# xiexh20/CHORE

Measured on AMD Instinct MI355X. Metric: query-points/sec (HGFilters encode + 20k-pt MLP field query per 512x512 image), higher is better.
Workload: dtype fp16x3; 1 GPU; BASELINE configs[1]: encode 4x(5,512,512) + query 4x20000 points per GPU per step; images_per_gpu=4, points_per_image=20000, batches_in_flight=2

## Files before the change

chore_amd/_lib.py:

```python
import ctypes
import os

import torch
from ctypes import POINTER, c_char_p, c_float, c_int, c_int64, c_longlong, c_size_t, c_uint8, c_void_p

_HERE = os.path.dirname(os.path.abspath(__file__))
LIB_PATH = os.environ.get("CHORE_HIP_LIB") or os.path.join(_HERE, "csrc", "libchore_hip.so")

F32, BF16, F16X3, F16 = 0, 1, 2, 3
HEADS_X3 = 0x100


class WeightDesc(ctypes.Structure):
    _fields_ = [("name", c_char_p), ("ptr", c_void_p), ("numel", c_int64)]


class EncoderCfg(ctypes.Structure):
    _fields_ = [("in_channels", c_int), ("num_stack", c_int), ("num_hourglass", c_int),
                ("hourglass_dim", c_int)]


SIGNATURES = {
    "chore_version": (c_int, []),
    "chore_create": (c_int, [POINTER(c_void_p), c_int]),
    "chore_destroy": (c_int, [c_void_p]),
    "chore_last_error": (c_char_p, [c_void_p]),
    "chore_cu_count": (c_int, [c_void_p]),
    "chore_stream_create_cu_mask": (c_int, [c_void_p, POINTER(ctypes.c_uint32), c_int, POINTER(c_void_p)]),
    "chore_stream_destroy": (c_int, [c_void_p, c_void_p]),
    "chore_heads_arena_bytes": (c_size_t, [c_int]),
    "chore_heads_pack": (c_int, [c_void_p, POINTER(WeightDesc), c_int, c_int, c_void_p, c_void_p]),
    "chore_query_fwd": (c_int, [c_void_p, c_void_p, c_void_p, c_int, c_int,
                                c_void_p, c_int, c_int, c_void_p, c_int, c_int, c_int,
                                c_void_p, POINTER(c_float), c_void_p, c_void_p, c_void_p, c_void_p,
                                c_void_p, c_void_p]),
    "chore_query_fwd_workspace_bytes": (c_size_t, [c_int, c_int]),
    "chore_query_fwd_ws": (c_int, [c_void_p, c_void_p, c_void_p, c_int, c_int,
                                   c_void_p, c_int, c_int, c_void_p, c_int, c_int, c_int,
                                   c_void_p, POINTER(c_float), c_void_p, c_void_p, c_void_p, c_void_p,
                                   c_void_p, c_void_p, c_void_p]),
    "chore_sample_features": (c_int, [c_void_p, c_void_p, c_void_p, c_int, c_int,
                                      c_void_p, c_int, c_int, c_void_p, c_int, c_int, c_int,
                                      POINTER(c_float), c_void_p, c_void_p, c_void_p, c_void_p]),
    "chore_query_bwd_points": (c_int, [c_void_p, c_void_p, c_void_p, c_int, c_int,
                                       c_void_p, c_int, c_int, c_void_p, c_int, c_int, c_int,
                                       c_void_p, POINTER(c_float), c_void_p, c_void_p, c_void_p,
                                       c_void_p, c_void_p, c_void_p]),
    "chore_query_train_bytes": (c_size_t, [c_int, c_int]),
    "chore_query_fwd_train": (c_int, [c_void_p, c_void_p, c_void_p, c_int, c_int,
                                      c_void_p, c_int, c_int, c_void_p, c_int, c_int, c_int,
                                      c_void_p, POINTER(c_float), c_void_p, c_void_p, c_void_p, c_void_p,
                                      c_void_p, c_void_p, c_void_p]),
    "chore_query_bwd_train": (c_int, [c_void_p, c_void_p, c_void_p, c_int, c_int,
                                      c_void_p, c_int, c_int, c_void_p, c_int, c_int, c_int,
                                      c_void_p, POINTER(c_float), c_void_p, c_void_p, c_void_p,
                                      c_void_p, c_void_p, c_void_p, c_int, c_void_p]),
    "chore_scatter_features": (c_int, [c_void_p, c_void_p, c_void_p, c_int, c_int, c_int, c_int, c_int, c_int,
                                       POINTER(c_float), c_void_p, c_void_p, c_void_p, c_int, c_void_p]),
    "chore_encoder_arena_bytes": (c_size_t, [POINTER(EncoderCfg), c_int]),
    "chore_encoder_pack": (c_int, [c_void_p, POINTER(EncoderCfg), POINTER(WeightDesc), c_int, c_int,
                                   c_void_p, c_void_p]),
    "chore_encoder_workspace_bytes": (c_size_t, [POINTER(EncoderCfg), c_int, c_int, c_int, c_int]),
    "chore_encode_fwd": (c_int, [c_void_p, POINTER(EncoderCfg), c_void_p, c_int, c_int, c_int, c_int,
                                 c_void_p, c_void_p, c_size_t, POINTER(c_void_p), c_int, c_void_p,
                                 c_void_p, c_void_p]),
    "chore_smpl_arena_bytes": (c_size_t, [c_int, c_int, c_int]),
    "chore_smpl_workspace_bytes": (c_size_t, [c_int, c_int, c_int, c_int]),
    "chore_smpl_pack": (c_int, [c_void_p, c_int, c_int, c_int, c_void_p, c_void_p, c_void_p, c_void_p, c_void_p,
                                POINTER(c_int), c_void_p, c_void_p]),
    "chore_smpl_lbs_fwd": (c_int, [c_void_p, c_void_p, c_int, c_int, c_int, c_void_p, c_void_p, c_void_p, c_void_p,
                                   c_float, c_int, c_void_p, c_void_p, c_void_p, c_void_p, c_void_p, c_void_p]),
    "chore_smpl_lbs_bwd": (c_int, [c_void_p, c_void_p, c_int, c_int, c_int, c_void_p, c_float, c_int, c_void_p,
                                   c_void_p, c_void_p, c_void_p, c_void_p, c_void_p, c_void_p, c_void_p]),
    "chore_landmarks_fwd": (c_int, [c_void_p, c_void_p, c_void_p, c_int, c_int, c_int, c_void_p, c_void_p]),
    "chore_landmarks_bwd": (c_int, [c_void_p, c_void_p, c_void_p, c_int, c_int, c_int, c_void_p, c_void_p]),
    "chore_so3_aux_bytes": (c_size_t, [c_int]),
    "chore_so3_project_fwd": (c_int, [c_void_p, c_void_p, c_int, c_void_p, c_void_p, c_void_p]),
    "chore_so3_project_bwd": (c_int, [c_void_p, c_void_p, c_void_p, c_int, c_void_p, c_void_p]),
    "chore_conv2d_workspace_bytes": (c_size_t, [c_int, c_int, c_int, c_int]),
    "chore_gn_stats_bytes": (c_size_t, [c_int]),
    "chore_gn_stats": (c_int, [c_void_p, c_int, c_void_p, c_int, c_int, c_int, c_void_p, c_int, c_void_p]),
    "chore_gn_relu_fwd": (c_int, [c_void_p, c_int, c_void_p, c_void_p, c_void_p, c_void_p, c_void_p, c_int, c_int, c_int,
                                  c_void_p]),
    "chore_conv2d_fwd": (c_int, [c_void_p, c_int, c_int, c_void_p, c_int, c_int, c_int, c_int, c_void_p, c_void_p,
                                 c_void_p, c_void_p, c_void_p, c_int, c_void_p, c_void_p, c_void_p, c_void_p]),
    "chore_conv2d_pool_fwd": (c_int, [c_void_p, c_int, c_int, c_void_p, c_int, c_int, c_int, c_int, c_void_p, c_void_p,
                                      c_void_p, c_void_p, c_void_p, c_int, c_void_p, c_void_p, c_void_p, c_void_p, c_void_p,
                                      c_void_p, c_void_p]),
    "chore_amax_bytes": (c_size_t, []),
    "chore_absmax_f32": (c_int, [c_void_p, c_void_p, c_size_t, c_void_p, c_void_p]),
    "chore_conv2d_bwd_data": (c_int, [c_void_p, c_int, c_int, c_void_p, c_int, c_int, c_int, c_int, c_void_p, c_int,
                                      c_void_p, c_void_p, c_void_p, c_void_p]),
    "chore_conv2d_wgrad_workspace_bytes": (c_size_t, [c_int, c_int, c_int, c_int, c_int, c_int]),
    "chore_conv2d_bwd_weight": (c_int, [c_void_p, c_int, c_int, c_void_p, c_int, c_int, c_int, c_int, c_void_p, c_void_p,
                                        c_void_p, c_void_p, c_int, c_void_p, c_void_p, c_void_p, c_void_p, c_void_p]),
    "chore_convblock_saved_bytes": (c_size_t, [c_int, c_int, c_int, c_int, c_int, c_int]),
    "chore_convblock_out_stats_offset": (c_size_t, [c_int]),
    "chore_convblock_workspace_bytes": (c_size_t, [c_int, c_int, c_int, c_int, c_int, c_int]),
    "chore_convblock_grad_floats": (c_size_t, [c_int, c_int]),
    "chore_convblock_fwd": (c_int, [c_void_p, c_int, c_void_p, c_void_p, c_int, c_int, c_int, c_int, c_int, c_void_p, c_void_p,
                                    c_void_p, c_void_p, c_void_p, c_void_p, c_void_p, c_void_p, c_void_p]),
    "chore_convblock_bwd": (c_int, [c_void_p, c_int, c_void_p, c_void_p, c_void_p, c_int, c_int, c_int, c_int, c_int, c_void_p,
                                    c_void_p, c_void_p, c_void_p, c_void_p, c_void_p, c_void_p, c_void_p, c_void_p, c_void_p]),
    "chore_debug_nan_counts": (c_int, [c_void_p]),
    "chore_debug_last_conv": (c_int, [c_void_p, POINTER(c_int), c_int]),
    "chore_debug_last_wgrad": (c_int, [c_void_p, POINTER(c_int), c_int]),
    "chore_query_plan": (c_int, [c_int] * 9 + [POINTER(c_int), c_int]),
    "chore_conv_plan": (c_int, [c_int] * 9 + [POINTER(c_int), c_int]),
    "chore_fit_adam_step": (c_int, [c_void_p, c_void_p, c_void_p, c_void_p, c_void_p, c_void_p, c_int, c_void_p, c_float, c_float,
                                    c_float, c_float, c_void_p, c_void_p]),
    "chore_fit_adam_step_acc": (c_int, [c_void_p, c_void_p, c_void_p, c_void_p, c_void_p, c_void_p, c_void_p, c_void_p, c_void_p, c_int,
                                        c_void_p, c_float, c_float, c_float, c_float, c_void_p, c_int, c_void_p]),
    "chore_fit_weighted_sum_step": (c_int, [c_void_p, c_void_p, c_void_p, c_int, c_void_p, c_void_p, c_void_p, c_void_p, c_void_p, c_void_p,
                                            c_void_p, c_void_p, c_float, c_void_p, c_void_p, c_void_p]),
    "chore_fit_weighted_sum": (c_int, [c_void_p, c_void_p, c_void_p, c_int, c_void_p, c_void_p, c_void_p]),
    "chore_fit_weighted_sum_bwd": (c_int, [c_void_p, c_void_p, c_int, c_void_p, c_void_p, c_void_p, c_void_p]),
    "chore_fit_smpl_terms_fwd": (c_int, [c_void_p] * 11 + [c_int, c_int, c_int, c_void_p, c_void_p, c_void_p]),
    "chore_fit_smpl_terms_bwd": (c_int, [c_void_p] * 11 + [c_int, c_int, c_int, c_void_p, c_void_p, c_void_p, c_void_p, c_void_p]),
    "chore_fit_point_terms_workspace_bytes": (c_size_t, [c_int, c_int]),
    "chore_fit_point_terms_fwd": (c_int, [c_void_p, c_void_p, c_int, c_float, c_void_p, c_void_p, c_int, c_int, c_int, c_void_p,
                                          c_void_p, c_void_p, c_void_p]),
    "chore_fit_point_terms_bwd": (c_int, [c_void_p, c_void_p, c_int, c_float, c_void_p, c_void_p, c_int, c_int, c_int, c_void_p,
                                          c_void_p, c_void_p, c_void_p, c_void_p]),
    "chore_fit_obj_transform_fwd": (c_int, [c_void_p] * 5 + [c_int, c_int, c_void_p, c_void_p]),
    "chore_fit_obj_transform_bwd": (c_int, [c_void_p] * 6 + [c_int, c_int, c_void_p, c_void_p, c_void_p, c_void_p]),
    "chore_fit_obj_terms_workspace_bytes": (c_size_t, [c_int]),
    "chore_fit_obj_terms_fwd": (c_int, [c_void_p] * 5 + [c_float, c_int, c_int, c_void_p, c_void_p, c_void_p, c_void_p, c_void_p]),
    "chore_fit_obj_terms_bwd": (c_int, [c_void_p, c_void_p, c_void_p, c_float, c_void_p, c_void_p, c_int, c_int, c_void_p, c_void_p,
                                        c_void_p, c_void_p]),
    "chore_fit_rot_noise": (c_int, [c_void_p, c_void_p, c_void_p, c_void_p, c_float, c_int, c_longlong, c_void_p, c_void_p]),
    "chore_fit_stop_rule": (c_int, [c_void_p, c_void_p, c_void_p, c_void_p, c_void_p, c_float, c_void_p, c_void_p, c_void_p]),
    "chore_train_loss_workspace_bytes": (c_size_t, []),
    "chore_train_loss": (c_int, [c_void_p] * 11 + [c_int, c_int, c_float, c_void_p, c_float] + [c_void_p] * 5 + [c_int, c_void_p,
                                                                                                               c_void_p]),
    "chore_upadd_fwd": (c_int, [c_void_p, c_int, c_void_p, c_void_p, c_void_p, c_int, c_int, c_int, c_int, c_void_p, c_void_p]),
    "chore_up2_bwd": (c_int, [c_void_p, c_int, c_void_p, c_void_p, c_int, c_int, c_int, c_int, c_void_p]),
    "chore_avgpool2_fwd": (c_int, [c_void_p, c_int, c_void_p, c_void_p, c_int, c_int, c_int, c_int, c_void_p, c_void_p]),
    "chore_avgpool2_bwd": (c_int, [c_void_p, c_int, c_void_p, c_void_p, c_int, c_int, c_int, c_int, c_void_p]),
    "chore_stem_workspace_bytes": (c_size_t, [c_int]),
    "chore_stem_fwd": (c_int, [c_void_p, c_int, c_void_p, c_int, c_int, c_int, c_int, c_void_p, c_void_p, c_void_p, c_void_p,
                               c_void_p]),
    "chore_stem_x3_workspace_bytes": (c_size_t, [c_int]),
    "chore_stem_x3_fwd": (c_int, [c_void_p, c_void_p, c_int, c_int, c_int, c_int, c_void_p, c_void_p, c_void_p, c_void_p, c_void_p,
                                  c_void_p]),
    "chore_stem_wgrad_workspace_bytes": (c_size_t, [c_int, c_int, c_int, c_int]),
    "chore_stem_bwd_weight": (c_int, [c_void_p, c_int, c_void_p, c_int, c_int, c_int, c_int, c_void_p, c_void_p, c_void_p,
                                      c_void_p, c_void_p]),
    "chore_heads_wgrad_floats": (c_size_t, []),
    "chore_heads_wgrad_workspace_bytes": (c_size_t, []),
    "chore_heads_wgrad": (c_int, [c_void_p, c_void_p, c_int, c_int, c_void_p, c_void_p, c_void_p, c_void_p, c_void_p, c_void_p,
                                  c_int, c_void_p]),
    "chore_gemm_tn_workspace_bytes": (c_size_t, [c_int, c_int, c_int]),
    "chore_gemm_tn_f32": (c_int, [c_void_p, c_void_p, c_int, c_void_p, c_int, c_int, c_int, c_int, c_void_p, c_void_p,
                                  c_void_p]),
    "chore_gn_relu_bwd_workspace_bytes": (c_size_t, [c_int, c_int]),
    "chore_gn_relu_bwd": (c_int, [c_void_p, c_int, c_void_p, c_void_p, c_void_p, c_void_p, c_void_p, c_int, c_int, c_int,
                                  c_void_p, c_void_p, c_void_p, c_void_p, c_int, c_void_p]),
    "chore_eval_chamfer_workspace_bytes": (c_size_t, [c_int, c_int]),
    "chore_eval_chamfer": (c_int, [c_void_p, c_void_p, c_int, c_void_p, c_int, c_void_p, c_void_p, c_void_p]),
    "chore_eval_procrustes": (c_int, [c_void_p, c_void_p, c_void_p, c_int, c_void_p, c_void_p]),
    "chore_eval_apply_similarity": (c_int, [c_void_p, c_void_p, c_int, c_void_p, c_void_p, c_void_p]),
    "chore_gen_clamp_mask": (c_int, [c_void_p, c_void_p, c_int, c_float, c_int, c_int, c_void_p, c_void_p]),
    "chore_gen_surface_step": (c_int, [c_void_p, c_void_p, c_void_p, c_void_p, c_int, c_float, c_int, c_int, c_void_p, c_void_p]),
    "chore_gen_surface_step_fused": (c_int, [c_void_p, c_void_p, c_void_p, c_int, c_int, c_void_p, c_int, c_int, c_void_p, c_int, c_int,
                                             c_int, c_void_p, POINTER(c_float), c_int, c_float, c_void_p, c_void_p]),
    "chore_gen_compact": (c_int, [c_void_p, c_void_p, c_int, c_int, c_void_p, c_void_p, c_void_p]),
# ... 160 lines not shown
```

chore_amd/csrc/enc_misc.hip:

```cpp
#include "enc_common.h"
#include <type_traits>
#include <cstdlib>

constexpr int STEM_T = 16;
constexpr int STEM_P = 2 * STEM_T + 5;
constexpr int STEM_MAXC = 8;

template <typename T>
__global__ __launch_bounds__(256) void stem_kernel(const float* __restrict__ img, int B, int Cin, int H, int W,
                                                   const float* __restrict__ wk, const float* __restrict__ bias,
                                                   T* __restrict__ out) {
    extern __shared__ __attribute__((aligned(16))) float sm[];
    float* patch = sm;
    const int OH = H / 2, OW = W / 2;
    const int b = blockIdx.z, ty0 = blockIdx.y * STEM_T, tx0 = blockIdx.x * STEM_T;
    const int tid = threadIdx.x;
    const int iy0 = 2 * ty0 - 3, ix0 = 2 * tx0 - 3;
    for (int i = tid; i < Cin * STEM_P * STEM_P; i += 256) {
        const int c = i / (STEM_P * STEM_P), r = i % (STEM_P * STEM_P);
        const int y = iy0 + r / STEM_P, x = ix0 + r % STEM_P;
        float v = 0.f;
        if (y >= 0 && y < H && x >= 0 && x < W) v = img[(((size_t)b * Cin + c) * H + y) * W + x];
        patch[i] = v;
    }
// ... 334 lines not shown
                           st);
    CHORE_LAUNCH_CHECK(h, s);
    return CHORE_OK;
}

template <typename T, bool STATS>
__global__ __launch_bounds__(256) void gn_apply_relu_kernel(const T* __restrict__ x, int xcs, int xco,
                                                            const GroupStat* __restrict__ st,
                                                            const float* __restrict__ gamma,
                                                            const float* __restrict__ beta, T* __restrict__ y,
                                                            int ycs, int yco, int C, int HW, GroupStat* __restrict__ st_out) {
    __shared__ float ss[512];
    __shared__ float red[STATS ? 2 : 1][STATS ? 1024 : 1];
    const int b = blockIdx.y, tid = threadIdx.x;
    if (tid < C) gn_scale_shift(st, (int)gridDim.y, b, C, tid, HW, gamma, beta, ss[2 * tid], ss[2 * tid + 1]);
    __syncthreads();
    const int tpr = C / 4;
    const size_t total4 = (size_t)HW * tpr;
    f32x4 sum = {0.f, 0.f, 0.f, 0.f}, sq = {0.f, 0.f, 0.f, 0.f};
    for (size_t i = (size_t)blockIdx.x * 256 + tid; i < total4; i += (size_t)gridDim.x * 256) {
        const int cv = (int)(i % tpr);
        const size_t p = (size_t)b * HW + i / tpr;
        const f32x4 v = Vec4<T>::ld(x + p * xcs + xco + cv * 4);
        f32x4 r;
#pragma unroll
        for (int j = 0; j < 4; ++j) {
            const float t = fmaf(v[j], ss[2 * (cv * 4 + j)], ss[2 * (cv * 4 + j) + 1]);
            r[j] = t > 0.f ? t : 0.f;
        }
        if constexpr (STATS) {
            const f32x4 w = Vec4<T>::st_round(y + p * ycs + yco + cv * 4, r);
            sum += w;
            sq += w * w;
        } else Vec4<T>::st(y + p * ycs + yco + cv * 4, r);
    }
    if constexpr (STATS) {
        const int cv = tid % tpr, pl = tid / tpr, P = 256 / tpr;
#pragma unroll
        for (int j = 0; j < 4; ++j) {
            red[0][pl * C + cv * 4 + j] = sum[j];
            red[1][pl * C + cv * 4 + j] = sq[j];
        }
        __syncthreads();
        if (tid < C) {
            float a = 0.f, q = 0.f;
            for (int i = 0; i < P; ++i) { a += red[0][i * C + tid]; q += red[1][i * C + tid]; }
            const int gs = C / GN_GROUPS;
            a = group_lane_sum(a, gs);
            q = group_lane_sum(q, gs);
            GroupStat* o = st_out + (size_t)b * GN_GROUPS + tid / gs;
            if (tid % gs == 0) stat_add(&o->sum, act_hi_cells((int)gridDim.y), a);
            if (tid % gs == (gs > 1 ? 1 : 0)) stat_add(&o->sq, act_hi_cells((int)gridDim.y), q);
        }
    }
}

int launch_gn_apply_relu(chore_handle* h, int dtype, const View& x, const GroupStat* st, const float* gamma,
                         const float* beta, const View& y, int B, int HW, hipStream_t s, GroupStat* st_out) {
    if (!gn_channels_ok(x.C)) CHORE_FAIL(h, CHORE_EINVAL, "gn: unsupported C=%d", x.C);
    const size_t total4 = (size_t)HW * (x.C / 4);
    int blocks = (int)((total4 + 255) / 256);
    if (blocks > 1024) blocks = 1024;
    if (st_out) {
        if (256 % (x.C / 4)) CHORE_FAIL(h, CHORE_EINVAL, "gn_apply_relu with statistics: unsupported C=%d", x.C);
        if (blocks > 256) blocks = 256;
    }
    dim3 grid(blocks, B);
#define GN_APPLY(T, ST) hipLaunchKernelGGL((gn_apply_relu_kernel<T, ST>), grid, dim3(256), 0, s, (const T*)x.p, x.cs, x.co, st, gamma, beta, \
                                            (T*)y.p, y.cs, y.co, x.C, HW, st_out)
    if (dtype == CHORE_F16) { if (st_out) GN_APPLY(h16_t, true); else GN_APPLY(h16_t, false); }
    else if (dtype == CHORE_F32) { if (st_out) GN_APPLY(float, true); else GN_APPLY(float, false); }
    else { if (st_out) GN_APPLY(bf16_t, true); else GN_APPLY(bf16_t, false); }
#undef GN_APPLY
    CHORE_LAUNCH_CHECK(h, s);
    return CHORE_OK;
}

constexpr int MAP_T = 8;

template <typename T, int C> struct PoolOp {
    const T* x; int xcs, xco, H, W;
    static constexpr size_t SMEM = 0;
    static constexpr int CT = C, TW = MAP_T;
    __device__ __forceinline__ void stage(char*, int, int, int, int, int, int) const {}
    __device__ __forceinline__ void column(const char*, int b, int oy0, int ox, int, int c0, int cv, int OH,
                                           f32x4 (&out)[MAP_T]) const {
#pragma unroll
        for (int r = 0; r < MAP_T; ++r) {
            const int oy = oy0 + r < OH ? oy0 + r : OH - 1;
            const T* src = x + (((size_t)b * H + 2 * oy) * W + 2 * ox) * xcs + xco + c0 + cv * 4;
            const f32x4 a = Vec4<T>::ld(src), bb = Vec4<T>::ld(src + xcs);
            const f32x4 c = Vec4<T>::ld(src + (size_t)W * xcs), d = Vec4<T>::ld(src + (size_t)W * xcs + xcs);
            out[r] = (((a + bb) + c) + d) * 0.25f;
        }
    }
};

__device__ __forceinline__ void cubic_coeffs(float t, float (&c)[4]) {
    const float A = -0.75f;
    const float x0 = t + 1.0f, x1 = t, x2 = 1.0f - t, x3 = 2.0f - t;
    c[0] = ((A * x0 - 5.0f * A) * x0 + 8.0f * A) * x0 - 4.0f * A;
    c[1] = ((A + 2.0f) * x1 - (A + 3.0f)) * x1 * x1 + 1.0f;
    c[2] = ((A + 2.0f) * x2 - (A + 3.0f)) * x2 * x2 + 1.0f;
    c[3] = ((A * x3 - 5.0f * A) * x3 + 8.0f * A) * x3 - 4.0f * A;
}
template <typename T, int C> struct UpAddOp {
    static constexpr int CT = 64, TW = 16;
    static constexpr int PS = 8, PSX = TW / 2 + 4;
    static constexpr int TPR = CT / 4, P = 256 / TPR;
    static constexpr size_t SMEM = (size_t)PS * PSX * CT * sizeof(T);
    static_assert(C % CT == 0 && (PS * PSX) % P == 0 && TW % P == 0, "upadd tile geometry");
    const T* a; int acs, aco;
    const T* low; int lcs, lco, H, W;
    __device__ __forceinline__ float scale_y() const { return (float)(H - 1) / (float)(2 * H - 1); }
    __device__ __forceinline__ float scale_x() const { return (float)(W - 1) / (float)(2 * W - 1); }
    __device__ __forceinline__ void stage(char* sm, int b, int oy0, int ox0, int c0, int cv, int pl) const {
        const int iy0 = (int)floorf(scale_y() * (float)oy0) - 1, ix0 = (int)floorf(scale_x() * (float)ox0) - 1;
        constexpr int N = PS * PSX / P;
        typedef typename std::conditional<sizeof(T) == 2, unsigned long long, f32x4>::type Raw;
        Raw v[N];
#pragma unroll
        for (int i = 0; i < N; ++i) {
            const int q = pl + i * P;
            int yy = iy0 + q / PSX, xx = ix0 + q % PSX;
            yy = yy < 0 ? 0 : (yy > H - 1 ? H - 1 : yy);
            xx = xx < 0 ? 0 : (xx > W - 1 ? W - 1 : xx);
            v[i] = *(const Raw*)(low + (((size_t)b * H + yy) * W + xx) * lcs + lco + c0 + cv * 4);
        }
#pragma unroll
        for (int i = 0; i < N; ++i) *(Raw*)((T*)sm + (size_t)(pl + i * P) * CT + cv * 4) = v[i];
    }
    __device__ __forceinline__ void column(const char* sm, int b, int oy0, int ox, int ox0, int c0, int cv, int OH,
                                           f32x4 (&out)[MAP_T]) const {
        const int OW = 2 * W;
        const int iy0 = (int)floorf(scale_y() * (float)oy0) - 1, ix0 = (int)floorf(scale_x() * (float)ox0) - 1;
        f32x4 av[MAP_T];
#pragma unroll
        for (int r = 0; r < MAP_T; ++r) {
            const int oy = oy0 + r < OH ? oy0 + r : OH - 1;
            av[r] = Vec4<T>::ld(a + (((size_t)b * 2 * H + oy) * OW + ox) * acs + aco + c0 + cv * 4);
        }
        const float rx = scale_x() * (float)ox, fx = floorf(rx);
        const int kx = (int)fx - 1 - ix0;
        float cx[4];
        cubic_coeffs(rx - fx, cx);
        f32x4 rows[PS];
#pragma unroll
        for (int k = 0; k < PS; ++k) {
            const T* pr = (const T*)sm + (size_t)(k * PSX + kx) * CT + cv * 4;
            f32x4 acc = Vec4<T>::ld(pr) * cx[0];
#pragma unroll
            for (int q = 1; q < 4; ++q) {
                const f32x4 v = Vec4<T>::ld(pr + (size_t)q * CT);
#pragma unroll
                for (int e = 0; e < 4; ++e) acc[e] = fmaf(v[e], cx[q], acc[e]);
            }
            rows[k] = acc;
        }
#pragma unroll
        for (int r = 0; r < MAP_T; ++r) {
            const int oy = oy0 + r < OH ? oy0 + r : OH - 1;
            const float ry = scale_y() * (float)oy, fy = floorf(ry);
            const int ky = (int)fy - 1 - iy0;
            float cy[4];
            cubic_coeffs(ry - fy, cy);
            f32x4 acc = {0.f, 0.f, 0.f, 0.f};
            bool first = true;
#pragma unroll
            for (int k = 0; k < PS; ++k) {
                const int j = k - ky;
                if (j >= 0 && j < 4) {
                    const float w = cy[j];
#pragma unroll
                    for (int e = 0; e < 4; ++e) acc[e] = first ? rows[k][e] * w : fmaf(rows[k][e], w, acc[e]);
                    first = false;
                }
            }
            out[r] = av[r] + acc;
        }
    }
};

template <typename T, int C, typename Op>
__global__ __launch_bounds__(256) void map_stats_kernel(Op op, T* y, int ycs, int yco, int OH, int OW,
                                                        GroupStat* __restrict__ st) {
    extern __shared__ __attribute__((aligned(16))) char map_sm[];
    __shared__ float red[2][1024];
    constexpr int CT = Op::CT, TW = Op::TW;
    constexpr int TPR = CT / 4, P = 256 / TPR;
    static_assert(P * CT <= 1024, "partial-sum scratch");
    const int b = blockIdx.y, tid = threadIdx.x, c0 = blockIdx.z * CT;
    const int cv = tid % TPR, pl = tid / TPR;
    const int tiles_x = (OW + TW - 1) / TW;
    const int oy0 = (blockIdx.x / tiles_x) * MAP_T, ox0 = (blockIdx.x % tiles_x) * TW;
    op.stage(map_sm, b, oy0, ox0, c0, cv, pl);
    __syncthreads();
    f32x4 sum = {0.f, 0.f, 0.f, 0.f}, sq = {0.f, 0.f, 0.f, 0.f};
#pragma unroll
    for (int col = pl; col < TW; col += P) {
        const int ox = ox0 + col;
        if (ox < OW) {
            f32x4 out[MAP_T];
            op.column(map_sm, b, oy0, ox, ox0, c0, cv, OH, out);
#pragma unroll
            for (int r = 0; r < MAP_T; ++r) {
                const int oy = oy0 + r;
                if (oy < OH) {
                    const f32x4 v = Vec4<T>::st_round(y + (((size_t)b * OH + oy) * OW + ox) * ycs + yco + c0 + cv * 4, out[r]);
                    sum += v;
                    sq += v * v;
                }
            }
        }
    }
    if (!st) return;
#pragma unroll
    for (int j = 0; j < 4; ++j) {
        red[0][pl * CT + cv * 4 + j] = sum[j];
        red[1][pl * CT + cv * 4 + j] = sq[j];
    }
    __syncthreads();
    if (tid < CT) {
        float a = 0.f, q = 0.f;
#pragma unroll
        for (int i = 0; i < P; ++i) { a += red[0][i * CT + tid]; q += red[1][i * CT + tid]; }
        constexpr int gs = C / GN_GROUPS;
        static_assert(CT % gs == 0, "a channel slice holds whole GroupNorm groups");
        a = group_lane_sum(a, gs);
        q = group_lane_sum(q, gs);
        GroupStat* o = st + (size_t)b * GN_GROUPS + (c0 + tid) / gs;
        if (tid % gs == 0) stat_add(&o->sum, act_hi_cells((int)gridDim.y), a);
        if (tid % gs == (gs > 1 ? 1 : 0)) stat_add(&o->sq, act_hi_cells((int)gridDim.y), q);
    }
}

template <typename T, int C, typename Op>
static int launch_map_c(chore_handle* h, const Op& op, const View& y, int B, int OH, int OW, GroupStat* st,
                        hipStream_t s) {
    dim3 grid(((OH + MAP_T - 1) / MAP_T) * ((OW + Op::TW - 1) / Op::TW), B, C / Op::CT);
    return CHORE_LAUNCH(h, s, (map_stats_kernel<T, C, Op>), grid, dim3(256), Op::SMEM, op, (T*)y.p, y.cs, y.co, OH, OW, st);
}

template <typename T>
static int launch_pool_t(chore_handle* h, const View& x, const View& y, int B, int H, int W, GroupStat* st,
                         hipStream_t s) {
    switch (y.C) {
        case 64: return launch_map_c<T, 64>(h, PoolOp<T, 64>{(const T*)x.p, x.cs, x.co, H, W}, y, B, H / 2, W / 2, st, s);
        case 128: return launch_map_c<T, 128>(h, PoolOp<T, 128>{(const T*)x.p, x.cs, x.co, H, W}, y, B, H / 2, W / 2, st, s);
        case 256: return launch_map_c<T, 256>(h, PoolOp<T, 256>{(const T*)x.p, x.cs, x.co, H, W}, y, B, H / 2, W / 2, st, s);
    }
    CHORE_FAIL(h, CHORE_EINVAL, "avgpool2: unsupported C=%d (64, 128, 256)", y.C);
}

int launch_avgpool2(chore_handle* h, int dtype, const View& x, const View& y, int B, int H, int W, GroupStat* st,
                    hipStream_t s) {
    if (dtype == CHORE_F16) return launch_pool_t<h16_t>(h, x, y, B, H, W, st, s);
    return dtype == CHORE_F32 ? launch_pool_t<float>(h, x, y, B, H, W, st, s)
                              : launch_pool_t<bf16_t>(h, x, y, B, H, W, st, s);
}

template <typename T>
static int launch_upadd_t(chore_handle* h, const View& a, const View& low, const View& y, int B, int H, int W,
                          GroupStat* st, hipStream_t s) {
    switch (y.C) {
        case 64: return launch_map_c<T, 64>(h, UpAddOp<T, 64>{(const T*)a.p, a.cs, a.co, (const T*)low.p, low.cs, low.co, H, W}, y, B, 2 * H, 2 * W, st, s);
        case 128: return launch_map_c<T, 128>(h, UpAddOp<T, 128>{(const T*)a.p, a.cs, a.co, (const T*)low.p, low.cs, low.co, H, W}, y, B, 2 * H, 2 * W, st, s);
        case 256: return launch_map_c<T, 256>(h, UpAddOp<T, 256>{(const T*)a.p, a.cs, a.co, (const T*)low.p, low.cs, low.co, H, W}, y, B, 2 * H, 2 * W, st, s);
    }
    CHORE_FAIL(h, CHORE_EINVAL, "upadd: unsupported C=%d (64, 128, 256)", y.C);
}

int launch_upadd(chore_handle* h, int dtype, const View& a, const View& low, const View& y, int B, int H, int W,
                 GroupStat* st, hipStream_t s) {
    if (dtype == CHORE_F16) return launch_upadd_t<h16_t>(h, a, low, y, B, H, W, st, s);
    return dtype == CHORE_F32 ? launch_upadd_t<float>(h, a, low, y, B, H, W, st, s)
                              : launch_upadd_t<bf16_t>(h, a, low, y, B, H, W, st, s);
}

__global__ void copy_f32_kernel(const float* __restrict__ src, float* __restrict__ dst, size_t n) {
    const size_t i = (size_t)blockIdx.x * 256 + threadIdx.x;
    if (i < n) dst[i] = src[i];
}
int launch_copy_f32(chore_handle* h, const float* src, float* dst, size_t n, hipStream_t s) {
    hipLaunchKernelGGL(copy_f32_kernel, dim3((unsigned)((n + 255) / 256)), dim3(256), 0, s, src, dst, n);
    CHORE_LAUNCH_CHECK(h, s);
    return CHORE_OK;
// ... 111 lines not shown
```

chore_amd/csrc/ops.hip:

```cpp
#include "enc_common.h"

extern "C" {

size_t chore_conv2d_workspace_bytes(int dtype, int taps, int Cin, int Cout) {
    if ((dtype != CHORE_F32 && dtype != CHORE_BF16 && dtype != CHORE_F16X3 && dtype != CHORE_F16) || (taps != 1 && taps != 9)) return 0;
    return packed_conv_bytes(dtype, taps, Cin, Cout);
}

size_t chore_gn_stats_bytes(int B) { return act_stats_bytes(B); }

size_t chore_amax_bytes(void) { return AMAX_CELLS * sizeof(unsigned); }
int chore_absmax_f32(chore_handle* h, const float* x, size_t n, void* amax, chore_stream_t stream) {
    CHORE_ENTER(h);
    return launch_absmax_f32(h, x, n, (unsigned*)amax, (hipStream_t)stream);
}
static inline int elem_dtype(int dtype) { return dtype == CHORE_F16X3 ? CHORE_F32 : dtype; }

int chore_gn_stats(chore_handle* h, int dtype, const void* x, int B, int HW, int C, void* stats, int zeroed,
                   chore_stream_t stream) {
    CHORE_ENTER(h);
    if (!x || !stats || B <= 0 || HW <= 0) CHORE_FAIL(h, CHORE_EINVAL, "chore_gn_stats: bad argument");
    dtype = elem_dtype(dtype);
    if (dtype != CHORE_F32 && dtype != CHORE_BF16 && dtype != CHORE_F16) CHORE_FAIL(h, CHORE_EINVAL, "chore_gn_stats: dtype");
    if (!gn_channels_ok(C)) CHORE_FAIL(h, CHORE_EINVAL, "chore_gn_stats: unsupported C=%d", C);
    hipStream_t s = (hipStream_t)stream;
    if (!zeroed) CHORE_HIP_CHECK(h, hipMemsetAsync(stats, 0, chore_gn_stats_bytes(B), s));
    View v; v.p = const_cast<void*>(x); v.cs = C; v.co = 0; v.C = C;
    return launch_gn_stats(h, dtype, v, B, HW, (GroupStat*)stats, s);
}

int chore_gn_relu_fwd(chore_handle* h, int dtype, const void* x, const void* stats, const float* gamma, const float* beta,
                      void* y, int B, int HW, int C, chore_stream_t stream) {
    CHORE_ENTER(h);
    if (!x || !stats || !gamma || !beta || !y) CHORE_FAIL(h, CHORE_EINVAL, "chore_gn_relu_fwd: null argument");
    if (B <= 0 || HW <= 0) CHORE_FAIL(h, CHORE_EINVAL, "chore_gn_relu_fwd: bad shape");
    dtype = elem_dtype(dtype);
    if (dtype != CHORE_F32 && dtype != CHORE_BF16 && dtype != CHORE_F16) CHORE_FAIL(h, CHORE_EINVAL, "chore_gn_relu_fwd: dtype");
    if (!gn_channels_ok(C)) CHORE_FAIL(h, CHORE_EINVAL, "chore_gn_relu_fwd: unsupported C=%d", C);
    View vx; vx.p = const_cast<void*>(x); vx.cs = C; vx.co = 0; vx.C = C;
    View vy; vy.p = y; vy.cs = C; vy.co = 0; vy.C = C;
    return launch_gn_apply_relu(h, dtype, vx, (const GroupStat*)stats, gamma, beta, vy, B, HW, (hipStream_t)stream);
}

int chore_conv2d_fwd(chore_handle* h, int dtype, int taps, const void* x, int B, int H, int W, int Cin,
                     const void* stats, const float* gamma, const float* beta, const float* w, const float* bias,
                     int Cout, void* y, void* out_stats, void* workspace, chore_stream_t stream) {
    CHORE_ENTER(h);
    if (!x || !w || !y || !workspace) CHORE_FAIL(h, CHORE_EINVAL, "chore_conv2d_fwd: null argument");
    if (stats && (!gamma || !beta)) CHORE_FAIL(h, CHORE_EINVAL, "chore_conv2d_fwd: GroupNorm needs gamma and beta");
    hipStream_t s = (hipStream_t)stream;
    int rc = launch_pack_conv(h, dtype, taps, Cin, Cout, w, workspace, s, 0);
    if (rc) return rc;
    ConvArgs a{};
    a.in.p = const_cast<void*>(x); a.in.cs = Cin; a.in.co = 0; a.in.C = Cin;
    a.in_st = (const GroupStat*)stats; a.gamma = gamma; a.beta = beta;
    a.wpk = workspace; a.bias = bias;
    a.out.p = y; a.out.cs = Cout; a.out.co = 0; a.out.C = Cout;
    a.B = B; a.H = H; a.W = W; a.Cout = Cout;
    if (out_stats) { a.st_out = (GroupStat*)out_stats; a.st_out_C = Cout; a.st_out_co = 0; }
    return launch_conv(h, dtype, taps, a, s);
}

int chore_conv2d_pool_fwd(chore_handle* h, int dtype, int taps, const void* x, int B, int H, int W, int Cin,
                          const void* stats, const float* gamma, const float* beta, const float* w, const float* bias,
                          int Cout, const void* res, void* y, void* out_stats, void* y_pool, void* pool_stats, void* workspace,
                          chore_stream_t stream) {
    CHORE_ENTER(h);
    if (!x || !w || !y_pool || !workspace) CHORE_FAIL(h, CHORE_EINVAL, "chore_conv2d_pool_fwd: null argument");
    if (stats && (!gamma || !beta)) CHORE_FAIL(h, CHORE_EINVAL, "chore_conv2d_pool_fwd: GroupNorm needs gamma and beta");
    if (B <= 0 || H <= 0 || W <= 0 || (H & 1) || (W & 1)) CHORE_FAIL(h, CHORE_EINVAL, "chore_conv2d_pool_fwd: H and W must be even");
    hipStream_t s = (hipStream_t)stream;
    const bool fold = stats && conv_pool_covers(dtype, taps, Cin, Cout, H, W);
    if (!fold && !y) CHORE_FAIL(h, CHORE_EINVAL, "chore_conv2d_pool_fwd: this layer pools in a pass of its own, which needs y");
    int rc = launch_pack_conv(h, dtype, taps, Cin, Cout, w, workspace, s, 0);
    if (rc) return rc;
    ConvArgs a{};
    a.in.p = const_cast<void*>(x); a.in.cs = Cin; a.in.co = 0; a.in.C = Cin;
    a.in_st = (const GroupStat*)stats; a.gamma = gamma; a.beta = beta;
    a.wpk = workspace; a.bias = bias;
    a.out.p = y; a.out.cs = Cout; a.out.co = 0; a.out.C = Cout;
    if (res) { a.res.p = const_cast<void*>(res); a.res.cs = Cout; a.res.co = 0; a.res.C = Cout; }
    a.B = B; a.H = H; a.W = W; a.Cout = Cout;
    if (out_stats && y) { a.st_out = (GroupStat*)out_stats; a.st_out_C = Cout; a.st_out_co = 0; }
    View vp; vp.p = y_pool; vp.cs = Cout; vp.co = 0; vp.C = Cout;
    if (fold) {
        a.pool = vp;
        if (pool_stats) { a.st_pool = (GroupStat*)pool_stats; a.st_pool_C = Cout; a.st_pool_co = 0; }
        return launch_conv(h, dtype, taps, a, s);
    }
    rc = launch_conv(h, dtype, taps, a, s);
    if (rc) return rc;
    const int edt = elem_dtype(dtype);
    if (edt != CHORE_F32 && edt != CHORE_BF16) CHORE_FAIL(h, CHORE_EINVAL, "chore_conv2d_pool_fwd: dtype");
    return launch_avgpool2(h, edt, a.out, vp, B, H, W, (GroupStat*)pool_stats, s);
}

int chore_conv2d_bwd_data(chore_handle* h, int dtype, int taps, const void* dy, int B, int H, int W, int Cout,
                          const float* w, int Cin, void* dx, void* workspace, const void* dy_amax, chore_stream_t stream) {
    CHORE_ENTER(h);
    if (!dy || !w || !dx || !workspace) CHORE_FAIL(h, CHORE_EINVAL, "chore_conv2d_bwd_data: null argument");
    if (dtype == CHORE_F16X3 && !dy_amax) CHORE_FAIL(h, CHORE_EINVAL, "chore_conv2d_bwd_data: the fp16 x 3 mode needs the range of dy (dy_amax)");
    hipStream_t s = (hipStream_t)stream;
    int rc = launch_pack_conv(h, dtype, taps,  Cout,  Cin, w, workspace, s, 1);
    if (rc) return rc;
    ConvArgs a{};
    a.in.p = const_cast<void*>(dy); a.in.cs = Cout; a.in.co = 0; a.in.C = Cout;
    a.wpk = workspace;
    a.out.p = dx; a.out.cs = Cin; a.out.co = 0; a.out.C = Cin;
    a.B = B; a.H = H; a.W = W; a.Cout = Cin;
    if (dtype == CHORE_F16X3) a.in_amax = (const unsigned*)dy_amax;
    return launch_conv(h, dtype, taps, a, s);
}

size_t chore_stem_workspace_bytes(int Cin) { return Cin > 0 ? (size_t)Cin * 49 * 64 * sizeof(float) : 0; }

int chore_stem_fwd(chore_handle* h, int dtype, const float* images, int B, int Cin, int H, int W, const float* w,
                   const float* bias, void* y, void* workspace, chore_stream_t stream) {
    CHORE_ENTER(h);
    if (!images || !w || !bias || !y || !workspace) CHORE_FAIL(h, CHORE_EINVAL, "chore_stem_fwd: null argument");
    if (B <= 0 || Cin <= 0 || H <= 0 || W <= 0 || (H & 1) || (W & 1)) CHORE_FAIL(h, CHORE_EINVAL, "chore_stem_fwd: bad shape");
    dtype = elem_dtype(dtype);
    if (dtype != CHORE_F32 && dtype != CHORE_BF16) CHORE_FAIL(h, CHORE_EINVAL, "chore_stem_fwd: dtype");
    hipStream_t s = (hipStream_t)stream;
    int rc = launch_pack_stem(h, Cin, w, (float*)workspace, s);
// ... 59 lines not shown
```

include/chore_hip.h:

```cpp
#ifndef CHORE_HIP_H
#define CHORE_HIP_H

#include <stddef.h>
#include <stdint.h>

#ifdef __cplusplus
extern "C" {
#endif

typedef struct chore_handle chore_handle;
typedef void* chore_stream_t;

enum {
    CHORE_OK = 0,
    CHORE_EINVAL = -1,
    CHORE_EHIP = -2,
    CHORE_ESTATE = -3,
    CHORE_ENOMEM = -4
};

enum { CHORE_F32 = 0, CHORE_BF16 = 1, CHORE_F16X3 = 2, CHORE_F16 = 3 };
enum { CHORE_HEADS_X3 = 0x100 };

typedef struct {
// ... 180 lines not shown
    const float* pts, const float* point_rgb, const float* radius, float radius_px, int N, float point_depth_bias,
    int size, int ssaa, float ambient, float near_z, float far_z, float tex_eps, const float* background3,
    const int* face_group, int face_layers,
    float* rgb, float* depth, float* alpha, int* sample_id, void* workspace, chore_stream_t stream);

size_t chore_instances_workspace_bytes(int B, int F, int G, int size, int ssaa);
int chore_instances_fwd(chore_handle* h, const float* tri, const int* face_group, int B, int F, int G, int size, int ssaa,
                        float near_z, float far_z, float* visible, float* full, int* face_samples, int* group_samples,
                        int* sample_face_index, void* workspace, chore_stream_t stream);

int chore_photo_textures_fwd(chore_handle* h, const float* tri, const float* depth, const float* photo,
                             const float* fallback, int B, int F, int ts, int S, int Hp, int Wp,
                             float near_z, float far_z, float depth_bias, int align_corners,
                             float* textures, unsigned char* texel_visible, chore_stream_t stream);
int chore_point_visibility(chore_handle* h, const float* pts, const float* depth, int B, int N, int S,
                           float near_z, float far_z, float depth_bias, int* visible, chore_stream_t stream);

int chore_load_textures(chore_handle* h, const float* uv, const int* face_image, const float* face_color,
                        const unsigned char* images, size_t images_bytes, const long long* image_off,
                        const int* image_hw, int M, int F, int ts, int wrapping, int bilinear, float* textures,
                        chore_stream_t stream);
int chore_texture_atlas_size(int F, int tso, int* height, int* width);
int chore_texture_atlas(chore_handle* h, const float* textures, int F, int tsi, int tso, float* image,
                        chore_stream_t stream);

size_t chore_eval_chamfer_workspace_bytes(int Nx, int Ny);
int chore_eval_chamfer(chore_handle* h, const double* x, int Nx, const double* y, int Ny, double* out, void* workspace,
                       chore_stream_t stream);
int chore_eval_procrustes(chore_handle* h, const double* S1, const double* S2, int N, double* params,
                          chore_stream_t stream);
int chore_eval_apply_similarity(chore_handle* h, const double* pts, int N, const double* params, double* out,
                                chore_stream_t stream);

int chore_gen_compact(chore_handle* h, const unsigned char* mask, int B, int N, int* order, int* counts,
                      chore_stream_t stream);
int chore_gen_append(chore_handle* h, const float* src, long long ss_b, long long ss_c, long long ss_n, const int* order,
                     const int* counts, const int* offsets, float* dst, long long ds_b, long long ds_c, long long ds_n,
                     int B, int C, int N, int cap, chore_stream_t stream);
int chore_gen_advance(chore_handle* h, const int* counts, int B, int* offsets, int* total, chore_stream_t stream);
int chore_gen_resample(chore_handle* h, const float* samples, int B, int N, const int* order, const int* counts,
                       const float* init, int Ninit, const float* u, const float* noise, int M, float sigma, float* out,
                       chore_stream_t stream);
int chore_gen_clamp_mask(chore_handle* h, const float* df, int k, float thr, int B, int N, float* g, chore_stream_t stream);
int chore_gen_surface_step(chore_handle* h, const float* points, const float* grad, const float* df, int k, float thr, int B,
                           int N, float* out, chore_stream_t stream);
int chore_gen_surface_step_fused(chore_handle* h, const float* points, const float* crop_center, int B, int N,
                                 const void* feat, int FH, int FW, const void* tmpx, int TH, int TW, int dtype,
                                 const void* heads_arena, const float* cam6_host, int k, float thr, float* out_points,
                                 chore_stream_t stream);

int chore_prep_masks2bbox(chore_handle* h, const unsigned char* mask0, const unsigned char* mask1, int H, int W, int thres,
                          int* bbox4, chore_stream_t stream);
int chore_prep_resize_u8(chore_handle* h, const unsigned char* src, int sh, int sw, int C, unsigned char* dst, int dh, int dw,
                         chore_stream_t stream);
int chore_prep_crop_compose(chore_handle* h, const unsigned char* rgb, const unsigned char* person_mask,
                            const unsigned char* obj_mask, int H, int W, int tl_x, int tl_y, int br_x, int br_y, int S,
                            float* images, chore_stream_t stream);
int chore_prep_crop_compose_mean(chore_handle* h, const unsigned char* rgb, const unsigned char* person_mask,
                                 const unsigned char* obj_mask, int H, int W, double cc_x, double cc_y, double mean_x, double mean_y,
                                 int tl_x, int tl_y, int br_x, int br_y, int S, float* images, chore_stream_t stream);

int chore_prep_blur_max_radius(void);
size_t chore_prep_blur_workspace_bytes(int B, int H, int W, int C);
int chore_prep_blur_u8(chore_handle* h, const unsigned char* src, int B, int H, int W, int C, const int* params, int max_r,
                       unsigned char* dst, void* workspace, chore_stream_t stream);
int chore_prep_train_compose(chore_handle* h, const unsigned char* rgb, const unsigned char* person_mask,
                             const unsigned char* obj_mask, int B, int H, int W, const int* tlbr_host, const int* flip_host,
                             int S, float* images, chore_stream_t stream);

size_t chore_collision_workspace_bytes(int B, int V, int F);
int chore_collision_fwd(chore_handle* h, const float* verts, const int* faces, int B, int V, int F, float* loss,
                        float* gverts, int* counts, void* workspace, chore_stream_t stream);
int chore_collision_bwd(chore_handle* h, const float* gverts, const float* gout, int B, int V, float* dverts,
                        chore_stream_t stream);

size_t chore_conv2d_workspace_bytes(int dtype, int taps, int Cin, int Cout);
size_t chore_gn_stats_bytes(int B);
size_t chore_amax_bytes(void);
int chore_absmax_f32(chore_handle* h, const float* x, size_t n, void* amax, chore_stream_t stream);
int chore_gn_stats(chore_handle* h, int dtype, const void* x, int B, int HW, int C, void* stats, int zeroed,
                   chore_stream_t stream);
int chore_gn_relu_fwd(chore_handle* h, int dtype, const void* x, const void* stats, const float* gamma,
                      const float* beta, void* y, int B, int HW, int C, chore_stream_t stream);
int chore_conv2d_fwd(chore_handle* h, int dtype, int taps, const void* x, int B, int H, int W, int Cin,
                     const void* stats, const float* gamma, const float* beta, const float* w, const float* bias,
                     int Cout, void* y, void* out_stats, void* workspace, chore_stream_t stream);
int chore_conv2d_pool_fwd(chore_handle* h, int dtype, int taps, const void* x, int B, int H, int W, int Cin,
                          const void* stats, const float* gamma, const float* beta, const float* w, const float* bias,
                          int Cout, const void* res, void* y, void* out_stats, void* y_pool, void* pool_stats, void* workspace,
                          chore_stream_t stream);
int chore_conv2d_bwd_data(chore_handle* h, int dtype, int taps, const void* dy, int B, int H, int W, int Cout,
                          const float* w, int Cin, void* dx, void* workspace, const void* dy_amax, chore_stream_t stream);
size_t chore_conv2d_wgrad_workspace_bytes(int taps, int B, int H, int W, int Cin, int Cout);
int chore_conv2d_bwd_weight(chore_handle* h, int dtype, int taps, const void* x, int B, int H, int W, int Cin,
                            const void* stats, const float* gamma, const float* beta, const void* dy, int Cout,
                            float* dw, float* dbias, void* workspace, const void* dy_amax, chore_stream_t stream);
size_t chore_gn_relu_bwd_workspace_bytes(int B, int C);
int chore_gn_relu_bwd(chore_handle* h, int dtype, const void* x, const void* stats, const float* gamma,
                      const float* beta, const void* da, int B, int HW, int C, void* dx, float* dgamma,
                      float* dbeta, void* workspace, int workspace_zeroed, chore_stream_t stream);
size_t chore_convblock_saved_bytes(int dtype, int B, int H, int W, int Cin, int Cout);
size_t chore_convblock_out_stats_offset(int B);
size_t chore_convblock_workspace_bytes(int dtype, int B, int H, int W, int Cin, int Cout);
size_t chore_convblock_grad_floats(int Cin, int Cout);
int chore_convblock_fwd(chore_handle* h, int dtype, const void* x, const void* x_stats, int B, int H, int W, int Cin,
                        int Cout, const float* w1, const float* w2, const float* w3, const float* wd,
                        const float* const* gb, void* y, void* saved, void* workspace, chore_stream_t stream);
int chore_convblock_bwd(chore_handle* h, int dtype, const void* x, const void* x_stats, const void* dy, int B, int H,
                        int W, int Cin, int Cout, const float* w1, const float* w2, const float* w3, const float* wd,
                        const float* const* gb, const void* saved, void* dx, float* grads, void* workspace,
                        chore_stream_t stream);
size_t chore_train_loss_workspace_bytes(void);
int chore_train_loss(chore_handle* h, const float* df, const float* pca, const float* parts, const float* centers,
                     const float* df_h, const float* df_o, const int64_t* parts_gt, const float* pca_gt,
                     const float* body_center, const float* obj_center, int B, int N, float max_dist,
                     const float* weights, float scale, float* g_df, float* g_pca, float* g_parts, float* g_centers,
                     float* losses, int accumulate, void* workspace, chore_stream_t stream);
int chore_upadd_fwd(chore_handle* h, int dtype, const void* a, const void* low, void* y, int B, int H, int W, int C,
                    void* out_stats, chore_stream_t stream);
int chore_up2_bwd(chore_handle* h, int dtype, const void* dy, void* dlow, int B, int H, int W, int C,
                  chore_stream_t stream);
int chore_avgpool2_fwd(chore_handle* h, int dtype, const void* x, void* y, int B, int H, int W, int C, void* out_stats,
                       chore_stream_t stream);
int chore_avgpool2_bwd(chore_handle* h, int dtype, const void* dy, void* dx, int B, int H, int W, int C,
                       chore_stream_t stream);
size_t chore_stem_workspace_bytes(int Cin);
int chore_stem_fwd(chore_handle* h, int dtype, const float* images, int B, int Cin, int H, int W, const float* w,
                   const float* bias, void* y, void* workspace, chore_stream_t stream);
size_t chore_stem_x3_workspace_bytes(int Cin);
int chore_stem_x3_fwd(chore_handle* h, const float* images, int B, int Cin, int H, int W, const float* w, const float* bias,
                      void* y, void* out_stats, void* workspace, chore_stream_t stream);
size_t chore_stem_wgrad_workspace_bytes(int B, int Cin, int H, int W);
int chore_stem_bwd_weight(chore_handle* h, int dtype, const float* images, int B, int Cin, int H, int W, const void* dy,
                          float* dw, float* dbias, void* workspace, chore_stream_t stream);
size_t chore_gemm_tn_workspace_bytes(int P, int M, int N);
int chore_gemm_tn_f32(chore_handle* h, const float* A, int lda, const float* B, int ldb, int P, int M, int N,
                      float* C, void* workspace, chore_stream_t stream);

int chore_profile_enable(chore_handle* h, int on);
int chore_profile_read(chore_handle* h, int max_classes, const char** names, double* ms, double* flops,
                       double* bytes, int64_t* launches);

int chore_fit_adam_step(chore_handle* h, float* const* p, const float* const* g, float* const* m, float* const* v,
                        const int* n, int nt, const float* step, float lr, float beta1, float beta2, float eps,
                        const uint8_t* stop, chore_stream_t stream);
int chore_fit_adam_step_acc(chore_handle* h, float* const* p, float* const* g, const float* const* gnew, float* const* m,
                            float* const* v, const int* n, const int* cols, const int* pstride, int nt, const float* step,
                            float lr, float beta1, float beta2, float eps, const uint8_t* stop, int step_counted,
                            chore_stream_t stream);
int chore_fit_stop_rule(chore_handle* h, const float* loss, float* prev, uint8_t* stop, const uint8_t* armed, float tol,
                        float* loss_out, float* step, chore_stream_t stream);
int chore_fit_weighted_sum(chore_handle* h, const float* const* losses, const float* coeffs, int n, const float* denom,
                           float* out, chore_stream_t stream);
int chore_fit_weighted_sum_bwd(chore_handle* h, const float* coeffs, int n, const float* denom, const float* g, float* grads,
                               chore_stream_t stream);
int chore_fit_weighted_sum_step(chore_handle* h, const float* const* losses, const float* coeffs, int n, const float* denom,
                                float* out, const float* seed, float* grads, float* prev, uint8_t* stop, uint8_t* frozen,
                                const uint8_t* armed, float tol, float* loss_out, float* step, chore_stream_t stream);

int chore_fit_smpl_terms_fwd(chore_handle* h, const float* pose, const float* pose_init, const float* J, const float* kpts,
                             const float* crop_center, const float* body_mean, const float* body_prec, const float* hand_mean,
                             const float* lhand_prec, const float* rhand_prec, int B, int P, int R, const float* cam8,
                             float* const* out5, chore_stream_t stream);
int chore_fit_smpl_terms_bwd(chore_handle* h, const float* pose, const float* pose_init, const float* J, const float* kpts,
                             const float* crop_center, const float* body_mean, const float* body_prec, const float* hand_mean,
                             const float* lhand_prec, const float* rhand_prec, int B, int P, int R, const float* cam8,
// ... 45 lines not shown
```

Before: 21.55 million points/s.

## Split map-kernel staging into load/store, prefetch skip input, flatten grid, specialize cubic rows

The pool/upsample map kernel now loads its shared-memory patch into registers, issues the skip-connection loads for every column before storing the patch, and only then synchronises, so global loads overlap. The vertical bicubic accumulation is replaced by a switch over compile-time row offsets, removing predicated per-row loops. The grid index is flattened with channel slices innermost, so neighbouring blocks read the same spatial tile. A new exported gn_relu_stats_fwd entry point returns output group stats alongside the GN+ReLU, at the cost of more live registers.

```diff
diff --git a/chore_amd/_lib.py b/chore_amd/_lib.py
--- a/chore_amd/_lib.py
+++ b/chore_amd/_lib.py
@@ -82,6 +82,8 @@
     "chore_gn_stats": (c_int, [c_void_p, c_int, c_void_p, c_int, c_int, c_int, c_void_p, c_int, c_void_p]),
     "chore_gn_relu_fwd": (c_int, [c_void_p, c_int, c_void_p, c_void_p, c_void_p, c_void_p, c_void_p, c_int, c_int, c_int,
                                   c_void_p]),
+    "chore_gn_relu_stats_fwd": (c_int, [c_void_p, c_int, c_void_p, c_void_p, c_void_p, c_void_p, c_void_p, c_void_p, c_int, c_int,
+                                        c_int, c_void_p]),
     "chore_conv2d_fwd": (c_int, [c_void_p, c_int, c_int, c_void_p, c_int, c_int, c_int, c_int, c_void_p, c_void_p,
                                  c_void_p, c_void_p, c_void_p, c_int, c_void_p, c_void_p, c_void_p, c_void_p]),
     "chore_conv2d_pool_fwd": (c_int, [c_void_p, c_int, c_int, c_void_p, c_int, c_int, c_int, c_int, c_void_p, c_void_p,
diff --git a/chore_amd/csrc/enc_misc.hip b/chore_amd/csrc/enc_misc.hip
--- a/chore_amd/csrc/enc_misc.hip
+++ b/chore_amd/csrc/enc_misc.hip
@@ -440,8 +440,12 @@
     const T* x; int xcs, xco, H, W;
     static constexpr size_t SMEM = 0;
     static constexpr int CT = C, TW = MAP_T;
-    __device__ __forceinline__ void stage(char*, int, int, int, int, int, int) const {}
-    __device__ __forceinline__ void column(const char*, int b, int oy0, int ox, int, int c0, int cv, int OH,
+    struct Patch {};
+    struct Pre {};
+    __device__ __forceinline__ void stage_load(int, int, int, int, int, int, Patch&) const {}
+    __device__ __forceinline__ void prefetch(int, int, int, int, int, int, int, Pre&) const {}
+    __device__ __forceinline__ void stage_store(char*, int, int, const Patch&) const {}
+    __device__ __forceinline__ void column(const char*, const Pre&, int b, int oy0, int ox, int, int c0, int cv, int OH,
                                            f32x4 (&out)[MAP_T]) const {
 #pragma unroll
         for (int r = 0; r < MAP_T; ++r) {
@@ -472,32 +476,46 @@
     const T* low; int lcs, lco, H, W;
     __device__ __forceinline__ float scale_y() const { return (float)(H - 1) / (float)(2 * H - 1); }
     __device__ __forceinline__ float scale_x() const { return (float)(W - 1) / (float)(2 * W - 1); }
-    __device__ __forceinline__ void stage(char* sm, int b, int oy0, int ox0, int c0, int cv, int pl) const {
+    typedef typename std::conditional<sizeof(T) == 2, unsigned long long, f32x4>::type Raw;
+    static constexpr int N = PS * PSX / P;
+    struct Patch { Raw v[N]; };
+    struct Pre { f32x4 av[MAP_T]; };
+    __device__ __forceinline__ void stage_load(int b, int oy0, int ox0, int c0, int cv, int pl, Patch& pt) const {
         const int iy0 = (int)floorf(scale_y() * (float)oy0) - 1, ix0 = (int)floorf(scale_x() * (float)ox0) - 1;
-        constexpr int N = PS * PSX / P;
-        typedef typename std::conditional<sizeof(T) == 2, unsigned long long, f32x4>::type Raw;
-        Raw v[N];
 #pragma unroll
         for (int i = 0; i < N; ++i) {
             const int q = pl + i * P;
             int yy = iy0 + q / PSX, xx = ix0 + q % PSX;
             yy = yy < 0 ? 0 : (yy > H - 1 ? H - 1 : yy);
             xx = xx < 0 ? 0 : (xx > W - 1 ? W - 1 : xx);
-            v[i] = *(const Raw*)(low + (((size_t)b * H + yy) * W + xx) * lcs + lco + c0 + cv * 4);
-        }
-#pragma unroll
-        for (int i = 0; i < N; ++i) *(Raw*)((T*)sm + (size_t)(pl + i * P) * CT + cv * 4) = v[i];
-    }
-    __device__ __forceinline__ void column(const char* sm, int b, int oy0, int ox, int ox0, int c0, int cv, int OH,
-                                           f32x4 (&out)[MAP_T]) const {
-        const int OW = 2 * W;
-        const int iy0 = (int)floorf(scale_y() * (float)oy0) - 1, ix0 = (int)floorf(scale_x() * (float)ox0) - 1;
-        f32x4 av[MAP_T];
+            pt.v[i] = *(const Raw*)(low + (((size_t)b * H + yy) * W + xx) * lcs + lco + c0 + cv * 4);
+        }
+    }
+    __device__ __forceinline__ void prefetch(int b, int oy0, int ox, int c0, int cv, int OH, int OW, Pre& pre) const {
 #pragma unroll
         for (int r = 0; r < MAP_T; ++r) {
             const int oy = oy0 + r < OH ? oy0 + r : OH - 1;
-            av[r] = Vec4<T>::ld(a + (((size_t)b * 2 * H + oy) * OW + ox) * acs + aco + c0 + cv * 4);
-        }
+            pre.av[r] = Vec4<T>::ld(a + (((size_t)b * OH + oy) * OW + ox) * acs + aco + c0 + cv * 4);
+        }
+    }
+    __device__ __forceinline__ void stage_store(char* sm, int cv, int pl, const Patch& pt) const {
+#pragma unroll
+        for (int i = 0; i < N; ++i) *(Raw*)((T*)sm + (size_t)(pl + i * P) * CT + cv * 4) = pt.v[i];
+    }
+    template <int KY> static __device__ __forceinline__ f32x4 vertical(const f32x4 (&rows)[PS], const float (&cy)[4]) {
+        static_assert(KY + 4 <= PS, "patch rows");
+        f32x4 acc;
+#pragma unroll
+        for (int e = 0; e < 4; ++e) acc[e] = rows[KY][e] * cy[0];
+#pragma unroll
+        for (int j = 1; j < 4; ++j)
+#pragma unroll
+            for (int e = 0; e < 4; ++e) acc[e] = fmaf(rows[KY + j][e], cy[j], acc[e]);
+        return acc;
+    }
+    __device__ __forceinline__ void column(const char* sm, const Pre& pre, int b, int oy0, int ox, int ox0, int c0, int cv, int OH,
+                                           f32x4 (&out)[MAP_T]) const {
+        const int iy0 = (int)floorf(scale_y() * (float)oy0) - 1, ix0 = (int)floorf(scale_x() * (float)ox0) - 1;
         const float rx = scale_x() * (float)ox, fx = floorf(rx);
         const int kx = (int)fx - 1 - ix0;
         float cx[4];
@@ -522,19 +540,15 @@
             const int ky = (int)fy - 1 - iy0;
             float cy[4];
             cubic_coeffs(ry - fy, cy);
-            f32x4 acc = {0.f, 0.f, 0.f, 0.f};
-            bool first = true;
-#pragma unroll
-            for (int k = 0; k < PS; ++k) {
-                const int j = k - ky;
-                if (j >= 0 && j < 4) {
-                    const float w = cy[j];
-#pragma unroll
-                    for (int e = 0; e < 4; ++e) acc[e] = first ? rows[k][e] * w : fmaf(rows[k][e], w, acc[e]);
-                    first = false;
-                }
-            }
-            out[r] = av[r] + acc;
+            f32x4 acc;
+            switch (ky) {
+                case 0: acc = vertical<0>(rows, cy); break;
+                case 1: acc = vertical<1>(rows, cy); break;
+                case 2: acc = vertical<2>(rows, cy); break;
+                case 3: acc = vertical<3>(rows, cy); break;
+                default: acc = vertical<4>(rows, cy); break;
+            }
+            out[r] = pre.av[r] + acc;
         }
     }
 };
@@ -547,19 +561,32 @@
     constexpr int CT = Op::CT, TW = Op::TW;
     constexpr int TPR = CT / 4, P = 256 / TPR;
     static_assert(P * CT <= 1024, "partial-sum scratch");
-    const int b = blockIdx.y, tid = threadIdx.x, c0 = blockIdx.z * CT;
+    const int tid = threadIdx.x;
+    constexpr int NS = C / CT;
+    const unsigned flat = blockIdx.x + gridDim.x * (blockIdx.y + gridDim.y * blockIdx.z);
+    const unsigned tile_b = flat / NS;
+    const int c0 = (int)(flat % NS) * CT, b = (int)(tile_b / gridDim.x), tile = (int)(tile_b % gridDim.x);
     const int cv = tid % TPR, pl = tid / TPR;
     const int tiles_x = (OW + TW - 1) / TW;
-    const int oy0 = (blockIdx.x / tiles_x) * MAP_T, ox0 = (blockIdx.x % tiles_x) * TW;
-    op.stage(map_sm, b, oy0, ox0, c0, cv, pl);
+    const int oy0 = (tile / tiles_x) * MAP_T, ox0 = (tile % tiles_x) * TW;
+    constexpr int NCOL = (TW + P - 1) / P;
+    typename Op::Patch patch;
+    typename Op::Pre pre[NCOL];
+    op.stage_load(b, oy0, ox0, c0, cv, pl, patch);
+#pragma unroll
+    for (int k = 0; k < NCOL; ++k) {
+        const int col = pl + k * P < TW ? pl + k * P : TW - 1;
+        op.prefetch(b, oy0, ox0 + col < OW ? ox0 + col : OW - 1, c0, cv, OH, OW, pre[k]);
+    }
+    op.stage_store(map_sm, cv, pl, patch);
     __syncthreads();
     f32x4 sum = {0.f, 0.f, 0.f, 0.f}, sq = {0.f, 0.f, 0.f, 0.f};
 #pragma unroll
-    for (int col = pl; col < TW; col += P) {
-        const int ox = ox0 + col;
-        if (ox < OW) {
+    for (int k = 0; k < NCOL; ++k) {
+        const int col = pl + k * P, ox = ox0 + col;
+        if (col < TW && ox < OW) {
             f32x4 out[MAP_T];
-            op.column(map_sm, b, oy0, ox, ox0, c0, cv, OH, out);
+            op.column(map_sm, pre[k], b, oy0, ox, ox0, c0, cv, OH, out);
 #pragma unroll
             for (int r = 0; r < MAP_T; ++r) {
                 const int oy = oy0 + r;
diff --git a/chore_amd/csrc/ops.hip b/chore_amd/csrc/ops.hip
--- a/chore_amd/csrc/ops.hip
+++ b/chore_amd/csrc/ops.hip
@@ -40,6 +40,19 @@
     View vx; vx.p = const_cast<void*>(x); vx.cs = C; vx.co = 0; vx.C = C;
     View vy; vy.p = y; vy.cs = C; vy.co = 0; vy.C = C;
     return launch_gn_apply_relu(h, dtype, vx, (const GroupStat*)stats, gamma, beta, vy, B, HW, (hipStream_t)stream);
+}
+
+int chore_gn_relu_stats_fwd(chore_handle* h, int dtype, const void* x, const void* stats, const float* gamma, const float* beta,
+                            void* y, void* out_stats, int B, int HW, int C, chore_stream_t stream) {
+    CHORE_ENTER(h);
+    if (!x || !stats || !gamma || !beta || !y || !out_stats) CHORE_FAIL(h, CHORE_EINVAL, "chore_gn_relu_stats_fwd: null argument");
+    if (B <= 0 || HW <= 0) CHORE_FAIL(h, CHORE_EINVAL, "chore_gn_relu_stats_fwd: bad shape");
+    dtype = elem_dtype(dtype);
+    if (dtype != CHORE_F32 && dtype != CHORE_BF16 && dtype != CHORE_F16) CHORE_FAIL(h, CHORE_EINVAL, "chore_gn_relu_stats_fwd: dtype");
+    if (!gn_channels_ok(C)) CHORE_FAIL(h, CHORE_EINVAL, "chore_gn_relu_stats_fwd: unsupported C=%d", C);
+    View vx; vx.p = const_cast<void*>(x); vx.cs = C; vx.co = 0; vx.C = C;
+    View vy; vy.p = y; vy.cs = C; vy.co = 0; vy.C = C;
+    return launch_gn_apply_relu(h, dtype, vx, (const GroupStat*)stats, gamma, beta, vy, B, HW, (hipStream_t)stream, (GroupStat*)out_stats);
 }
 
 int chore_conv2d_fwd(chore_handle* h, int dtype, int taps, const void* x, int B, int H, int W, int Cin,
diff --git a/include/chore_hip.h b/include/chore_hip.h
--- a/include/chore_hip.h
+++ b/include/chore_hip.h
@@ -286,6 +286,8 @@
                    chore_stream_t stream);
 int chore_gn_relu_fwd(chore_handle* h, int dtype, const void* x, const void* stats, const float* gamma,
                       const float* beta, void* y, int B, int HW, int C, chore_stream_t stream);
+int chore_gn_relu_stats_fwd(chore_handle* h, int dtype, const void* x, const void* stats, const float* gamma,
+                            const float* beta, void* y, void* out_stats, int B, int HW, int C, chore_stream_t stream);
 int chore_conv2d_fwd(chore_handle* h, int dtype, int taps, const void* x, int B, int H, int W, int Cin,
                      const void* stats, const float* gamma, const float* beta, const float* w, const float* bias,
                      int Cout, void* y, void* out_stats, void* workspace, chore_stream_t stream);
```

Measured after the change: 21.67 million points/s (median of 6 runs). No clear change (+0.6%).
